# MengRao/pollnet

Hardware: AMD Instinct MI355X
Metric: device-resident Gbit/s + Mframes/s, 1500 B IPv4/TCP frames, 1/2/4/8 MI355X (higher is better)
Workload: dtype u16/u32 integer (one's-complement sums)

## Files before the change

### pollnet_amd/csrc/rx_service.hip

```cpp
#include <algorithm>
#include <chrono>
#include <cstdlib>

#include "rx_classify.hpp"

namespace {
using pn_internal::hip_err;
using pn_internal::set_err;

struct alignas(64) SvcPost {
  uint32_t gen;
  uint32_t n;
  uint32_t fpw;
  uint32_t max_conn;
  const uint8_t* frames;
  pn_result* out;
  const pn_conn_entry* tbl;
  uint16_t* links;
  uint32_t mask;
  uint32_t n_entries;
  uint32_t check;
  uint32_t seq;
};
static_assert(sizeof(SvcPost) == 64, "one line per post");

constexpr uint32_t kDoneWords = 64;
constexpr uint32_t kCountWords = 64;
constexpr uint32_t kExitWord = 96;
constexpr uint32_t kWordsBytes = 512;
constexpr uint32_t kLatWaves = PN_SERVICE_WAVES;
static_assert(kLatWaves <= kDoneWords, "a latency-tier post completes through per-wave done words");
constexpr uint32_t kLatFrames = kLatWaves * kFramesPerWave;
constexpr uint32_t kNetLimitMs = 8000;
constexpr uint32_t kPostVerify = 1u << 30, kPostLinks = 1u << 29, kPostN = (1u << 21) - 1;
constexpr uint32_t kLinkFrames = PN_LINK_MAX_FRAMES, kLinkConns = PN_LINK_MAX_CONNS;
constexpr uint32_t kMailBytes = 4096;

struct alignas(64) SvcDev {
  uint32_t count[2][16];
};
constexpr uint32_t kExitFlag = 32;

#ifdef PN_SVC_TRACE
__device__ uint64_t* g_svc_trace = nullptr;
#define SVC_T(w, i)                                                       \
  do {                                                                    \
    if (lane == 0 && (w) < 64) g_svc_trace[(w) * 8 + (i)] = wall_clock64(); \
  } while (0)
#else
#define SVC_T(w, i) \
  do {              \
  } while (0)
#endif

struct SArgs {
  const SvcPost* mail;
  u32x4* scratch;
  uint32_t* done_words;
  uint32_t* exit_word;
  SvcDev* dev;
  uint64_t idle_ticks;
  uint64_t net_ticks;
  uint32_t epoch;
  uint32_t last;
  uint32_t stride, ipa_off, avail;
  uint32_t poll_sleep;
};

inline uint32_t svc_fpw(uint32_t n, bool verify) {
  uint32_t fpw = verify ? 8u : kFramesPerWave;
  while (fpw < kFramesPerWave && (n + fpw - 1) / fpw > kLatWaves) fpw <<= 1;
  return fpw;
}

inline uint32_t svc_check(const SvcPost* p, uint32_t k) {
  const uint32_t* w = reinterpret_cast<const uint32_t*>(p);
  uint32_t x = k;
  for (int i = 1; i <= 13; i++) x ^= w[i];
  return x;
}

__host__ __device__ __forceinline__ uint32_t svc_active(uint32_t n, uint32_t fpw, uint32_t waves) {
  const uint32_t groups = (n + fpw - 1) / fpw;
  return groups < waves ? groups : waves;
}

inline uint32_t svc_helpers(uint32_t n, uint32_t max) {
  if (n <= kLatFrames) return 0;
  const uint32_t groups = (n + kFramesPerWave - 1) / kFramesPerWave;
  return std::min(groups - kLatWaves, max);
}

__device__ __forceinline__ KArgsAux svc_args(uint32_t v, uint32_t b, const SArgs& s, uint32_t k) {
  auto w32 = [&](uint32_t i) { return (uint32_t)__builtin_amdgcn_readlane(v, b + i); };
  auto u64 = [&](uint32_t lo) { return ((uint64_t)w32(lo + 1) << 32) | w32(lo); };
  KArgsAux a;
  const uint32_t nw = w32(1);
  a.n = nw & kPostN;
  a.fpw = w32(2) & 0xffu;
  a.max_conn = w32(3);
  a.frames = reinterpret_cast<const uint8_t*>(u64(4));
  a.out = reinterpret_cast<pn_result*>(u64(6));
  a.tbl = reinterpret_cast<const pn_conn_entry*>(u64(8));
  a.mask = w32(12);
  a.n_entries = w32(13);
  a.stride = s.stride;
  a.ipa_off = s.ipa_off;
  a.avail = s.avail;
  a.offs = nullptr;
  a.aux = (nw & kPostLinks) ? s.scratch + (size_t)(k & 1) * kLinkFrames * 2 : nullptr;
  return a;
}

__device__ __forceinline__ uint16_t* svc_links(uint32_t v, uint32_t b) {
  return reinterpret_cast<uint16_t*>(((uint64_t)(uint32_t)__builtin_amdgcn_readlane(v, b + 11) << 32) |
                                     (uint32_t)__builtin_amdgcn_readlane(v, b + 10));
}

constexpr uint32_t kCleanNeed = PN_F_HIT | PN_F_ACK | PN_F_IP_OK;
constexpr uint32_t kCleanNone = PN_F_TW | PN_F_SYN | PN_F_FIN | PN_F_RST | PN_F_NOT_TCP | PN_F_TRUNC | PN_F_BADOFF |
                                PN_F_IHL_NE_5;

struct ChainLds {
  uint32_t last[kLinkConns];
  uint32_t key[kLinkFrames];
  uint32_t seq_end[kLinkFrames];
  u32x4 fields[kLinkFrames];
};

__device__ __forceinline__ ChainLds& chain_lds() {
  __shared__ ChainLds c;
  return c;
}

__device__ __forceinline__ void chain_init(int lane) {
  ChainLds& c = chain_lds();
  for (uint32_t i = lane; i < kLinkConns; i += kWave) c.last[i] = 0u;
  wave_lds_sync();
}

__device__ __forceinline__ void chain_step(ChainLds& c, uint32_t base, uint32_t n, uint32_t max_conn, bool on,
                                           const u32x4& rec, const u32x4& fx, const __amdgpu_buffer_rsrc_t& lr,
                                           uint64_t below, int lane) {
  const uint32_t i = base + lane;
  const bool valid = i < n;
  const uint32_t flags = rec.w & 0xffffu;
  const uint32_t len = rec.z >> 16;
  const bool member = on && valid && (flags & (PN_F_HIT | PN_F_TW)) == PN_F_HIT && rec.x < max_conn;
  const bool usable = (flags & kCleanNeed) == kCleanNeed && (flags & kCleanNone) == 0 &&
                      (flags & (PN_F_TCP_OK | PN_F_TCP_UNCHECKED)) != 0 && len != 0 && len < 0x8000u;
  const uint32_t key = member ? rec.x : 0u;
  if (valid) {
    c.key[i] = member ? key : 0xFFFFFFFFu;
    c.seq_end[i] = rec.y + len;
    c.fields[i] = u32x4{fx.x, fx.y, fx.z, (rec.z & 0xffffu) | (usable ? 0x10000u : 0u)};
  }
  uint32_t prev = 0;
  if (member) prev = c.last[key];
  wave_lds_sync();
  if (member) atomicMax(&c.last[key], i + 1);
  wave_lds_sync();
  uint64_t todo = __ballot(member && c.last[key] != i + 1);
  while (todo) {
    const uint32_t leader = (uint32_t)__builtin_ctzll(todo);
    const uint32_t kk = __builtin_amdgcn_readlane(key, leader);
    const uint64_t m = __ballot(member && key == kk);
    todo &= ~m;
    const uint64_t lower = m & below;
    if (member && key == kk && lower) prev = base + 64u - (uint32_t)__builtin_clzll(lower);
  }
  uint32_t d = 0;
  if (member && usable && prev) {
    const uint32_t j = prev - 1;
    const u32x4 pf = c.fields[j];
    if ((pf.w >> 16) && c.seq_end[j] == rec.y && pf.x == fx.x && pf.y == fx.y && pf.z == fx.z &&
        (pf.w & 0xffffu) == (rec.z & 0xffffu))
      d = i - j;
  }
  if (valid) __builtin_amdgcn_raw_buffer_store_b16((unsigned short)d, lr, i * 2, 0, 0);
  wave_lds_sync();
}

__device__ __forceinline__ void chain_pass(const u32x4* aux, uint32_t n, uint32_t max_conn, uint16_t* links, int lane) {
  constexpr int kChunk = 8;
  ChainLds& c = chain_lds();
  const bool on = max_conn <= kLinkConns;
  const __amdgpu_buffer_rsrc_t lr = frame_rsrc(reinterpret_cast<const uint8_t*>(links), n * 2);
  const __amdgpu_buffer_rsrc_t ar = frame_rsrc(reinterpret_cast<const uint8_t*>(aux), n * 32);
  const uint64_t below = (1ull << lane) - 1;
  for (uint32_t base0 = 0; base0 < n; base0 += kChunk * kWave) {
    u32x4 rec[kChunk], fx[kChunk];
#pragma unroll
    for (int s = 0; s < kChunk; ++s) {
      const uint32_t i = base0 + s * kWave + lane;
      rec[s] = __builtin_amdgcn_raw_buffer_load_b128(ar, i * 32, 0, 0);
      fx[s] = __builtin_amdgcn_raw_buffer_load_b128(ar, i * 32 + 16, 0, 0);
    }
#pragma unroll
    for (int s = 0; s < kChunk; ++s)
      if (base0 + s * kWave < n) chain_step(c, base0 + s * kWave, n, max_conn, on, rec[s], fx[s], lr, below, lane);
  }
  for (uint32_t i = lane; i < n; i += kWave) {
    const uint32_t k = c.key[i];
    if (k != 0xFFFFFFFFu) c.last[k] = 0u;
  }
  wave_lds_sync();
}

template <int MIS, int COOP, bool HELPER = false>
__device__ __forceinline__ void svc_run(const KArgsAux& a, bool verify, bool linked, uint32_t w, uint32_t act, uint32_t k,
                                        uint32_t* done_word, int lane) {
  for (uint32_t g = w; g * a.fpw < a.n; g += act) {
    if (verify) classify_group<MIS, COOP, kProdAbl | kChainAux, kLoadAux, kStoreAux, 0, kLoadAux>(a, g * a.fpw, lane);
    else
      classify_group<MIS, COOP, kProdAbl | kHeaderOnly | kChainAux, kLoadAux, kStoreAux, 0, kLoadAux>(a, g * a.fpw, lane);
  }
  if constexpr (HELPER) return;
  __threadfence_system();
  if (lane == 0 && act <= kDoneWords && !linked)
    __hip_atomic_store(done_word, k, __ATOMIC_RELAXED, __HIP_MEMORY_SCOPE_SYSTEM);
}

template <bool PASS>
__device__ __forceinline__ void svc_finish(const KArgsAux& a, uint16_t* links, uint32_t k, uint32_t* count_word, int lane) {
  if constexpr (PASS) {
    if (a.aux) {
      __builtin_amdgcn_fence(__ATOMIC_ACQUIRE, "agent");
      chain_pass(a.aux, a.n, a.max_conn, links, lane);
    }
  }
  __threadfence_system();
  if (lane == 0) __hip_atomic_store(count_word, k, __ATOMIC_RELAXED, __HIP_MEMORY_SCOPE_SYSTEM);
}

template <bool PASS>
__device__ __forceinline__ void svc_count(uint32_t* count, const KArgsAux& a, uint16_t* links, uint32_t target, uint32_t k,
                                          uint32_t* count_word, int lane) {
  uint32_t prev = 0;
  if (lane == 0) prev = atomicAdd(count, 1u);
  prev = __builtin_amdgcn_readfirstlane(prev);
  if (prev == target - 1) {
    if (lane == 0) __hip_atomic_store(count, 0u, __ATOMIC_RELAXED, __HIP_MEMORY_SCOPE_AGENT);
    svc_finish<PASS>(a, links, k, count_word, lane);
  }
}

template <int MIS, int COOP>
__global__ __launch_bounds__(kWave) void rx_service_kernel(SArgs s) {
  const int lane = threadIdx.x;
  const uint32_t w = blockIdx.x, W = gridDim.x;
  const uint32_t* mw = reinterpret_cast<const uint32_t*>(s.mail);
  uint32_t last = s.last;
  uint64_t t0 = wall_clock64();
  chain_init(lane);
  for (;;) {
    const uint32_t v = lane <= (int)kExitFlag ? __hip_atomic_load(mw + lane, __ATOMIC_RELAXED, __HIP_MEMORY_SCOPE_SYSTEM) : 0u;
    if (w != 0 && (uint32_t)__builtin_amdgcn_readlane(v, kExitFlag) == s.epoch) return;
    const uint32_t k = last + 1;
    const uint32_t b = (k & 1) * 16;
    const uint32_t q = __builtin_amdgcn_readlane(v, b + 15);
    uint32_t x = q;
#pragma unroll
    for (uint32_t i = 1; i <= 13; i++) x ^= (uint32_t)__builtin_amdgcn_readlane(v, b + i);
    const bool whole = (uint32_t)__builtin_amdgcn_readlane(v, b) == q && (uint32_t)__builtin_amdgcn_readlane(v, b + 14) == x;
    if (!whole || (int32_t)(q - k) < 0) {
      if (w == 0) {
        if (wall_clock64() - t0 > s.idle_ticks) {
          if (lane == 0) {
            __hip_atomic_store(const_cast<uint32_t*>(mw) + kExitFlag, s.epoch, __ATOMIC_RELAXED, __HIP_MEMORY_SCOPE_SYSTEM);
            __hip_atomic_store(s.exit_word, s.epoch, __ATOMIC_RELEASE, __HIP_MEMORY_SCOPE_SYSTEM);
          }
          return;
        }
        __builtin_amdgcn_s_sleep(1);
      } else {
        if (wall_clock64() - t0 > s.net_ticks) return;
        for (uint32_t i = 0; i < s.poll_sleep; ++i) __builtin_amdgcn_s_sleep(1);
      }
      continue;
    }
    if (q != k) {
      last = k;
      t0 = wall_clock64();
      continue;
    }
    const uint32_t nw = __builtin_amdgcn_readlane(v, b + 1);
    if (nw == PN_SERVICE_STOP) return;
    last = k;
    const uint32_t fw = __builtin_amdgcn_readlane(v, b + 2);
    const uint32_t act = svc_active(nw & kPostN, fw & 0xffu, W + (fw >> 8));
    if (w < act) {
      SVC_T(w, 0);
      __builtin_amdgcn_fence(__ATOMIC_ACQUIRE, "");
      SVC_T(w, 1);
      const KArgsAux a = svc_args(v, b, s, k);
      SVC_T(w, 5);
      const bool linked = a.aux != nullptr;
      svc_run<MIS, COOP>(a, (nw & kPostVerify) != 0, linked, w, act, k, s.done_words + w, lane);
      SVC_T(w, 6);
      if (act > kDoneWords || linked) {
        uint32_t* cw = s.done_words + kCountWords + (k & 1);
        if (act == 1) svc_finish<true>(a, svc_links(v, b), k, cw, lane);
        else svc_count<true>(&s.dev->count[k & 1][0], a, svc_links(v, b), act < W ? act : W, k, cw, lane);
      }
      SVC_T(w, 7);
    }
    t0 = wall_clock64();
  }
}

template <int MIS, int COOP>
__global__ __launch_bounds__(kWave) void rx_service_helper_kernel(KArgsAux a, uint32_t verify, uint32_t act) {
  svc_run<MIS, COOP, true>(a, verify != 0, false, kLatWaves + blockIdx.x, act, 0, nullptr, threadIdx.x);
}

template <int MIS>
void launch_svc(bool coop, uint32_t waves, const SArgs& a, hipStream_t s) {
  if (coop) hipLaunchKernelGGL((rx_service_kernel<MIS, 1>), dim3(waves), dim3(kWave), 0, s, a);
  else hipLaunchKernelGGL((rx_service_kernel<MIS, 0>), dim3(waves), dim3(kWave), 0, s, a);
}

template <int MIS>
void launch_helpers(bool coop, uint32_t helpers, const KArgsAux& a, uint32_t verify, uint32_t act, hipStream_t s) {
  if (coop) hipLaunchKernelGGL((rx_service_helper_kernel<MIS, 1>), dim3(helpers), dim3(kWave), 0, s, a, verify, act);
  else hipLaunchKernelGGL((rx_service_helper_kernel<MIS, 0>), dim3(helpers), dim3(kWave), 0, s, a, verify, act);
}
}

struct pn_service {
  pn_ctx* ctx = nullptr;
  hipStream_t stream = nullptr;
  hipStream_t helper_stream = nullptr;
  uint32_t stride = 0, frame_off = 0;
  uint32_t helpers_max = 0;
  uint32_t post_helpers[2] = {0, 0};
  hipEvent_t helper_ev[2] = {nullptr, nullptr};
  uint64_t idle_ticks = 0, net_ticks = 0;
  SvcPost* mail = nullptr;
  bool mail_dev = false;
  uint32_t* words = nullptr;
  uint32_t post_words[2] = {0, 0};
  uint32_t tbl_post[2] = {0, 0};
  bool tbl_used[2] = {false, false};
  SvcDev* dev = nullptr;
  u32x4* scratch = nullptr;
  uint32_t seq = 0;
  uint32_t epoch = 0;
  bool running = false;
  bool coop = false;
};

namespace {
SArgs svc_sargs(const pn_service* v, uint32_t base) {
  SArgs a;
  a.mail = v->mail;
  a.scratch = v->scratch;
  a.done_words = v->words;
  a.exit_word = v->words + kExitWord;
  a.dev = v->dev;
  a.idle_ticks = v->idle_ticks;
  a.net_ticks = v->net_ticks;
  a.epoch = v->epoch;
  a.last = base;
  a.stride = v->stride;
  a.ipa_off = (v->frame_off + 14) & ~15u;
  a.avail = v->stride - v->frame_off;
  a.poll_sleep = v->mail_dev ? 1u : 16u;
  return a;
}

inline void host_sfence() { asm volatile("sfence" ::: "memory"); }

void svc_publish(SvcPost* slot, const SvcPost& q, bool wc) {
  static const bool avx = __builtin_cpu_supports("avx");
  if (wc && avx) {
    asm volatile(
        "vmovdqu (%0), %%ymm0\n\t"
        "vmovdqu 32(%0), %%ymm1\n\t"
        "vmovntdq %%ymm0, (%1)\n\t"
        "vmovntdq %%ymm1, 32(%1)\n\t"
        "sfence\n\t"
        "vzeroupper"
        :
        : "r"(&q), "r"(slot)
        : "memory", "xmm0", "xmm1");
    return;
  }
  volatile uint32_t* d = reinterpret_cast<volatile uint32_t*>(slot);
  const uint32_t* w = reinterpret_cast<const uint32_t*>(&q);
  for (int i = 1; i <= 14; ++i) d[i] = w[i];
  host_sfence();
  d[0] = w[0];
  d[15] = w[15];
  host_sfence();
}

int svc_launch_helpers(pn_service* v, uint32_t k, uint32_t helpers, const SvcPost& q) {
  KArgsAux a;
  strided_kargs(a, q.frames, q.out, q.tbl, q.mask, q.n_entries, q.max_conn, q.n & kPostN, v->stride, v->frame_off);
  a.fpw = q.fpw & 0xffu;
  const uint32_t verify = (q.n & kPostVerify) ? 1u : 0u, act = svc_active(a.n, a.fpw, kLatWaves + helpers);
  hipStream_t s = v->helper_stream;
  for_mis(v->frame_off, [&](auto mis) { launch_helpers<mis()>(v->coop, helpers, a, verify, act, s); });
  hipError_t e = hipGetLastError();
  if (e == hipSuccess && !v->helper_ev[k & 1]) e = hipEventCreateWithFlags(&v->helper_ev[k & 1], hipEventDisableTiming);
  if (e == hipSuccess) e = hipEventRecord(v->helper_ev[k & 1], s);
  if (e != hipSuccess) return hip_err(v->ctx, e, "pn_service: helper launch");
  return PN_OK;
}

int svc_launch(pn_service* v, uint32_t base) {
  pn_ctx* ctx = v->ctx;
  const SvcDev init{};
  hipError_t e = hipMemcpyAsync(v->dev, &init, sizeof(SvcDev), hipMemcpyHostToDevice, v->stream);
  if (e == hipSuccess) e = hipStreamSynchronize(v->stream);
  if (e != hipSuccess) return hip_err(ctx, e, "pn_service: device state");
  if (++v->epoch == 0) ++v->epoch;
  const SArgs a = svc_sargs(v, base);
  for_mis(v->frame_off, [&](auto mis) { launch_svc<mis()>(v->coop, kLatWaves, a, v->stream); });
  e = hipGetLastError();
  if (e != hipSuccess) return hip_err(ctx, e, "pn_service: launch");
  v->running = true;
  return PN_OK;
}

bool svc_post_ran(const pn_service* v, uint32_t k) {
  const uint32_t words = v->post_words[k & 1];
  if (words == 0 && (int32_t)(__atomic_load_n(v->words + kCountWords + (k & 1), __ATOMIC_ACQUIRE) - k) < 0) return false;
  for (uint32_t w = 0; w < words; ++w)
    if ((int32_t)(__atomic_load_n(v->words + w, __ATOMIC_ACQUIRE) - k) < 0) return false;
  if (v->post_helpers[k & 1] && hipEventQuery(v->helper_ev[k & 1]) != hipSuccess) return false;
  return true;
}

bool svc_post_done(const pn_service* v, uint32_t k) {
  if ((int32_t)(v->seq - k) >= 2) return true;
  if (!svc_post_ran(v, k)) return false;
  return k != v->seq || svc_post_ran(v, k - 1);
}

uint32_t svc_done(const pn_service* v) {
  if (svc_post_done(v, v->seq)) return v->seq;
  return svc_post_done(v, v->seq - 1) ? v->seq - 1 : v->seq - 2;
}

bool svc_exited(const pn_service* v) { return __atomic_load_n(v->words + kExitWord, __ATOMIC_ACQUIRE) == v->epoch; }

void svc_free(pn_service* v) {
  if (v->ctx) {
    auto& l = v->ctx->services;
    l.erase(std::remove(l.begin(), l.end(), v), l.end());
  }
  if (v->mail) (void)(v->mail_dev ? hipFree(v->mail) : hipHostFree(v->mail));
  if (v->words) (void)hipHostFree(v->words);
  if (v->dev) (void)hipFree(v->dev);
  if (v->scratch) (void)hipFree(v->scratch);
  if (v->stream) (void)hipStreamDestroy(v->stream);
  if (v->helper_stream) (void)hipStreamDestroy(v->helper_stream);
  for (hipEvent_t ev : v->helper_ev)
    if (ev) (void)hipEventDestroy(ev);
  delete v;
}
}

int pn_internal::svc_release_table(pn_ctx* ctx, int buf) {
  for (pn_service* v : ctx->services) {
    if (!v->tbl_used[buf]) continue;
    const uint32_t id = v->tbl_post[buf];
    if ((int32_t)(v->seq - id) < 2 && !svc_post_done(v, id)) {
      const int rc = pn_service_wait(v, id);
      if (rc) return rc;
    }
    v->tbl_used[buf] = false;
  }
  return PN_OK;
}

extern "C" {

int pn_service_open(pn_ctx* ctx, uint32_t slot_stride, uint32_t frame_off, uint32_t idle_ms, pn_service** out) {
  return pn_service_open_ex(ctx, slot_stride, frame_off, idle_ms, 0, out);
}

int pn_service_open_ex(pn_ctx* ctx, uint32_t slot_stride, uint32_t frame_off, uint32_t idle_ms, uint32_t large_waves,
                       pn_service** out) {
  if (!ctx || !out) return set_err(ctx, PN_EINVAL, "pn_service_open: ctx / out is NULL");
  *out = nullptr;
  if ((slot_stride & 15) || slot_stride > 65536 || (frame_off & 1) || slot_stride < frame_off + 96)
    return set_err(ctx, PN_EINVAL, "pn_service_open: slot_stride/frame_off violate the layout contract");
  if (idle_ms == 0 || idle_ms > 10000) return set_err(ctx, PN_EINVAL, "pn_service_open: idle_ms must be in [1, 10000]");
  if (large_waves && (large_waves < PN_SERVICE_WAVES || large_waves > PN_SERVICE_MAX_WAVES))
    return set_err(ctx, PN_EINVAL, "pn_service_open: large_waves must be 0 or in [PN_SERVICE_WAVES, PN_SERVICE_MAX_WAVES]");
  hipError_t e = hipSetDevice(ctx->device);
  if (e != hipSuccess) return hip_err(ctx, e, "hipSetDevice");
  int khz = 0;
  e = hipDeviceGetAttribute(&khz, hipDeviceAttributeWallClockRate, ctx->device);
  if (e != hipSuccess || khz <= 0) return hip_err(ctx, e, "pn_service_open: wall clock rate");
  int cus = 0;
  e = hipDeviceGetAttribute(&cus, hipDeviceAttributeMultiprocessorCount, ctx->device);
  if (e != hipSuccess || cus <= 0) return hip_err(ctx, e, "pn_service_open: CU count");
  pn_service* v = new pn_service();
  v->ctx = ctx;
  v->stride = slot_stride;
  v->frame_off = frame_off;
  const uint32_t total = large_waves ? large_waves
                                     : std::max<uint32_t>(kLatWaves, std::min<uint32_t>(PN_SERVICE_MAX_WAVES,
                                                                                      (uint32_t)cus * PN_SERVICE_WAVES_PER_CU));
  v->helpers_max = total - kLatWaves;
  v->idle_ticks = (uint64_t)khz * idle_ms;
  v->net_ticks = v->idle_ticks + (v->idle_ticks >> 1) + (uint64_t)khz * kNetLimitMs;
  v->coop = (slot_stride % 16) == 0 && ((frame_off + 14) & ~15u) >= 16;
  int large_bar = 0;
  if (hipDeviceGetAttribute(&large_bar, hipDeviceAttributeIsLargeBar, ctx->device) != hipSuccess) large_bar = 0;
  v->mail_dev = large_bar != 0 && std::getenv("PN_SERVICE_HOST_MAILBOX") == nullptr;
  if (v->mail_dev && hipExtMallocWithFlags((void**)&v->mail, kMailBytes, hipDeviceMallocUncached) != hipSuccess) {
    (void)hipGetLastError();
    v->mail = nullptr;
    v->mail_dev = false;
  }
  if ((e = hipStreamCreateWithFlags(&v->stream, hipStreamNonBlocking)) != hipSuccess ||
      (e = hipStreamCreateWithFlags(&v->helper_stream, hipStreamNonBlocking)) != hipSuccess ||
      (!v->mail && (e = hipHostMalloc((void**)&v->mail, kMailBytes, hipHostMallocDefault)) != hipSuccess) ||
      (e = hipHostMalloc((void**)&v->words, kWordsBytes, hipHostMallocDefault)) != hipSuccess ||
      (e = hipMalloc((void**)&v->dev, sizeof(SvcDev))) != hipSuccess ||
      (e = hipMalloc((void**)&v->scratch, sizeof(u32x4) * 2 * 2 * kLinkFrames)) != hipSuccess) {
    const int rc = hip_err(ctx, e, "pn_service_open: allocation");
    svc_free(v);
    return rc;
  }
  uint32_t first = 0;
  if (const char* env = std::getenv("PN_SERVICE_FIRST_POST")) first = (uint32_t)std::strtoull(env, nullptr, 0);
  std::memset(v->words, 0, kWordsBytes);
  for (uint32_t w = 0; w < kDoneWords + 2; ++w) v->words[w] = first;
  {
    SvcPost q{};
    q.gen = q.seq = first;
    q.check = ~svc_check(&q, first);
    for (int i = 0; i < 2; ++i) svc_publish(v->mail + i, q, v->mail_dev);
    volatile uint32_t* flag = reinterpret_cast<volatile uint32_t*>(v->mail) + kExitFlag;
    *flag = 0u;
    host_sfence();
  }
  v->seq = first;
  const int rc = svc_launch(v, first);
  if (rc) {
    svc_free(v);
    return rc;
  }
  ctx->services.push_back(v);
  *out = v;
  return PN_OK;
}

int pn_service_post(pn_service* v, const void* frames, uint32_t n, void* results, uint32_t* post_id) {
  return pn_service_post_linked(v, frames, n, results, nullptr, post_id);
}

int pn_service_post_linked(pn_service* v, const void* frames, uint32_t n, void* results, uint16_t* links,
                           uint32_t* post_id) {
  if (!v) return set_err(nullptr, PN_EINVAL, "pn_service_post: service is NULL");
  pn_ctx* ctx = v->ctx;
  if (!ctx->tbl_dev) return set_err(ctx, PN_ENOTABLE, "pn_service_post: no conn table (call pn_set_conn_table)");
  if (n == 0 || n > PN_SERVICE_MAX_FRAMES || !frames || !results)
    return set_err(ctx, PN_EINVAL, "pn_service_post: n must be in [1, PN_SERVICE_MAX_FRAMES], buffers set");
  if (((uintptr_t)frames & 15) || ((uintptr_t)results & 15))
    return set_err(ctx, PN_EINVAL, "pn_service_post: frames/results must be 16-byte aligned");
  if (links && (n > PN_LINK_MAX_FRAMES || ((uintptr_t)links & 1)))
    return set_err(ctx, PN_EINVAL, "pn_service_post_linked: n must be <= PN_LINK_MAX_FRAMES, links 2-byte aligned");
  const uint32_t done = svc_done(v);
  if ((int32_t)(v->seq - done) >= 2) return set_err(ctx, PN_EINVAL, "pn_service_post: two posts already outstanding");
  if (v->running && svc_exited(v)) v->running = false;
  if (!v->running) {
    const int rc = svc_launch(v, done);
    if (rc) return rc;
  }
  const uint32_t k = v->seq + 1;
  const bool verify = ctx->verify_tcp;
  SvcPost q{};
  q.n = n | (verify ? kPostVerify : 0u) | (links ? kPostLinks : 0u);
  q.max_conn = ctx->max_conn;
  q.frames = (const uint8_t*)frames;
  q.out = (pn_result*)results;
  q.tbl = ctx->tbl_dev;
  q.links = links;
  q.mask = (uint32_t)ctx->mask;
  q.n_entries = ctx->n_entries;
  const uint32_t fpw = svc_fpw(n, verify), helpers = svc_helpers(n, v->helpers_max);
  q.fpw = fpw | helpers << 8;
  const uint32_t act = svc_active(n, fpw, kLatWaves + helpers);
  if (helpers) {
    const int rc = svc_launch_helpers(v, k, helpers, q);
    if (rc) return rc;
  }
  v->post_helpers[k & 1] = helpers;
  v->post_words[k & 1] = (act <= kDoneWords && !links) ? act : 0u;
  v->tbl_post[ctx->cur] = k;
  v->tbl_used[ctx->cur] = true;
  q.check = svc_check(&q, k);
  q.gen = q.seq = k;
  svc_publish(v->mail + (k & 1), q, v->mail_dev);
  v->seq = k;
  if (post_id) *post_id = k;
  return PN_OK;
}

int pn_service_wait(pn_service* v, uint32_t post_id) {
  if (!v) return set_err(nullptr, PN_EINVAL, "pn_service_wait: service is NULL");
  if (post_id == 0 || (int32_t)(post_id - v->seq) > 0 || (int32_t)(v->seq - post_id) >= 2)
    post_id = v->seq;
  const uint32_t k = post_id;
  const auto t_start = std::chrono::steady_clock::now();
  for (uint64_t i = 1;; ++i) {
    if (svc_post_done(v, k)) return PN_OK;
    if ((i & 4095) == 0) {
      if (std::chrono::steady_clock::now() - t_start > std::chrono::seconds(10))
        return set_err(v->ctx, PN_EHIP, "pn_service_wait: no completion within 10 s");
      if (svc_exited(v)) {
        const uint32_t done = svc_done(v);
        if ((int32_t)(done - k) >= 0) return PN_OK;
        v->running = false;
        const int rc = svc_launch(v, done);
        if (rc) return rc;
        continue;
      }
      const hipError_t q = hipStreamQuery(v->stream);
      if (q != hipErrorNotReady && q != hipSuccess) return hip_err(v->ctx, q, "pn_service_wait: the service kernel failed");
      if (q == hipSuccess && !svc_post_done(v, k) && !svc_exited(v))
        return set_err(v->ctx, PN_EHIP, "pn_service_wait: the service kernel ended without completing the post");
    }
  }
}

int pn_service_close(pn_service* v) {
  if (!v) return PN_OK;
  pn_ctx* ctx = v->ctx;
  int rc = svc_post_done(v, v->seq) ? PN_OK : pn_service_wait(v, 0);
  if (v->running && !svc_exited(v)) {
    const uint32_t k = v->seq + 1;
    SvcPost q{};
    q.n = PN_SERVICE_STOP;
    v->post_words[k & 1] = 0;
    v->post_helpers[k & 1] = 0;
    q.check = svc_check(&q, k);
    q.gen = q.seq = k;
    svc_publish(v->mail + (k & 1), q, v->mail_dev);
    v->seq = k;
  }
  hipError_t e = hipStreamSynchronize(v->stream);
  if (e == hipSuccess) e = hipStreamSynchronize(v->helper_stream);
  if (e != hipSuccess && rc == PN_OK) rc = hip_err(ctx, e, "pn_service_close");
  svc_free(v);
  return rc;
}

}

#ifdef PN_SVC_TRACE
extern "C" int pn_svc_trace_set(uint64_t* host_buf) {
  return hipMemcpyToSymbol(HIP_SYMBOL(g_svc_trace), &host_buf, sizeof host_buf) == hipSuccess ? PN_OK : PN_EHIP;
}
#endif
```

Before: 51120.

## Launch one helper block per frame group instead of a capped persistent helper grid

The helper kernel used to be a capped set of waves that each looped over frame groups in strided order. It now launches one block per remaining group, in slices, with XCD-aware group mapping and a higher occupancy launch bound. It also drops the chain-aux flag from helper classification and adds propagation of helper errors. The aim is to remove the loop overhead and load imbalance of the persistent helper waves, at the cost of more blocks and possibly several launches for very large posts.

Result: no change. 51120 (-0.0%).

```diff
diff --git a/pollnet_amd/csrc/rx_service.hip b/pollnet_amd/csrc/rx_service.hip
--- a/pollnet_amd/csrc/rx_service.hip
+++ b/pollnet_amd/csrc/rx_service.hip
@@ -85,10 +85,9 @@
   return groups < waves ? groups : waves;
 }
 
-inline uint32_t svc_helpers(uint32_t n, uint32_t max) {
-  if (n <= kLatFrames) return 0;
-  const uint32_t groups = (n + kFramesPerWave - 1) / kFramesPerWave;
-  return std::min(groups - kLatWaves, max);
+inline uint32_t svc_helpers(uint32_t n, bool tier_only) {
+  if (n <= kLatFrames || tier_only) return 0;
+  return (n + kFramesPerWave - 1) / kFramesPerWave - kLatWaves;
 }
 
 __device__ __forceinline__ KArgsAux svc_args(uint32_t v, uint32_t b, const SArgs& s, uint32_t k) {
@@ -207,7 +206,7 @@
   wave_lds_sync();
 }
 
-template <int MIS, int COOP, bool HELPER = false>
+template <int MIS, int COOP>
 __device__ __forceinline__ void svc_run(const KArgsAux& a, bool verify, bool linked, uint32_t w, uint32_t act, uint32_t k,
                                         uint32_t* done_word, int lane) {
   for (uint32_t g = w; g * a.fpw < a.n; g += act) {
@@ -215,7 +214,6 @@
     else
       classify_group<MIS, COOP, kProdAbl | kHeaderOnly | kChainAux, kLoadAux, kStoreAux, 0, kLoadAux>(a, g * a.fpw, lane);
   }
-  if constexpr (HELPER) return;
   __threadfence_system();
   if (lane == 0 && act <= kDoneWords && !linked)
     __hip_atomic_store(done_word, k, __ATOMIC_RELAXED, __HIP_MEMORY_SCOPE_SYSTEM);
@@ -310,8 +308,10 @@
 }
 
 template <int MIS, int COOP>
-__global__ __launch_bounds__(kWave) void rx_service_helper_kernel(KArgsAux a, uint32_t verify, uint32_t act) {
-  svc_run<MIS, COOP, true>(a, verify != 0, false, kLatWaves + blockIdx.x, act, 0, nullptr, threadIdx.x);
+__global__ __launch_bounds__(kWave, 4) void rx_service_helper_kernel(KArgs a, uint32_t verify, uint32_t first) {
+  const uint32_t base = (first + xcd_group(blockIdx.x, gridDim.x)) * a.fpw;
+  if (verify) classify_group<MIS, COOP, kProdAbl, kLoadAux, kStoreAux, 0, kLoadAux>(a, base, threadIdx.x);
+  else classify_group<MIS, COOP, kProdAbl | kHeaderOnly, kLoadAux, kStoreAux, 0, kLoadAux>(a, base, threadIdx.x);
 }
 
 template <int MIS>
@@ -321,9 +321,9 @@
 }
 
 template <int MIS>
-void launch_helpers(bool coop, uint32_t helpers, const KArgsAux& a, uint32_t verify, uint32_t act, hipStream_t s) {
-  if (coop) hipLaunchKernelGGL((rx_service_helper_kernel<MIS, 1>), dim3(helpers), dim3(kWave), 0, s, a, verify, act);
-  else hipLaunchKernelGGL((rx_service_helper_kernel<MIS, 0>), dim3(helpers), dim3(kWave), 0, s, a, verify, act);
+void launch_helpers(bool coop, uint32_t groups, const KArgs& a, uint32_t verify, uint32_t first, hipStream_t s) {
+  if (coop) hipLaunchKernelGGL((rx_service_helper_kernel<MIS, 1>), dim3(groups), dim3(kWave), 0, s, a, verify, first);
+  else hipLaunchKernelGGL((rx_service_helper_kernel<MIS, 0>), dim3(groups), dim3(kWave), 0, s, a, verify, first);
 }
 }
 
@@ -332,9 +332,10 @@
   hipStream_t stream = nullptr;
   hipStream_t helper_stream = nullptr;
   uint32_t stride = 0, frame_off = 0;
-  uint32_t helpers_max = 0;
+  uint32_t helper_slice = 0;
   uint32_t post_helpers[2] = {0, 0};
   hipEvent_t helper_ev[2] = {nullptr, nullptr};
+  mutable hipError_t helper_err = hipSuccess;
   uint64_t idle_ticks = 0, net_ticks = 0;
   SvcPost* mail = nullptr;
   bool mail_dev = false;
@@ -396,12 +397,15 @@
 }
 
 int svc_launch_helpers(pn_service* v, uint32_t k, uint32_t helpers, const SvcPost& q) {
-  KArgsAux a;
+  KArgs a;
   strided_kargs(a, q.frames, q.out, q.tbl, q.mask, q.n_entries, q.max_conn, q.n & kPostN, v->stride, v->frame_off);
   a.fpw = q.fpw & 0xffu;
-  const uint32_t verify = (q.n & kPostVerify) ? 1u : 0u, act = svc_active(a.n, a.fpw, kLatWaves + helpers);
+  const uint32_t verify = (q.n & kPostVerify) ? 1u : 0u;
   hipStream_t s = v->helper_stream;
-  for_mis(v->frame_off, [&](auto mis) { launch_helpers<mis()>(v->coop, helpers, a, verify, act, s); });
+  for (uint32_t g0 = 0; g0 < helpers; g0 += v->helper_slice) {
+    const uint32_t groups = std::min(v->helper_slice, helpers - g0);
+    for_mis(v->frame_off, [&](auto mis) { launch_helpers<mis()>(v->coop, groups, a, verify, kLatWaves + g0, s); });
+  }
   hipError_t e = hipGetLastError();
   if (e == hipSuccess && !v->helper_ev[k & 1]) e = hipEventCreateWithFlags(&v->helper_ev[k & 1], hipEventDisableTiming);
   if (e == hipSuccess) e = hipEventRecord(v->helper_ev[k & 1], s);
@@ -429,7 +433,13 @@
   if (words == 0 && (int32_t)(__atomic_load_n(v->words + kCountWords + (k & 1), __ATOMIC_ACQUIRE) - k) < 0) return false;
   for (uint32_t w = 0; w < words; ++w)
     if ((int32_t)(__atomic_load_n(v->words + w, __ATOMIC_ACQUIRE) - k) < 0) return false;
-  if (v->post_helpers[k & 1] && hipEventQuery(v->helper_ev[k & 1]) != hipSuccess) return false;
+  if (v->post_helpers[k & 1]) {
+    const hipError_t e = hipEventQuery(v->helper_ev[k & 1]);
+    if (e != hipSuccess) {
+      if (e != hipErrorNotReady) v->helper_err = e;
+      return false;
+    }
+  }
   return true;
 }
 
@@ -496,17 +506,11 @@
   int khz = 0;
   e = hipDeviceGetAttribute(&khz, hipDeviceAttributeWallClockRate, ctx->device);
   if (e != hipSuccess || khz <= 0) return hip_err(ctx, e, "pn_service_open: wall clock rate");
-  int cus = 0;
-  e = hipDeviceGetAttribute(&cus, hipDeviceAttributeMultiprocessorCount, ctx->device);
-  if (e != hipSuccess || cus <= 0) return hip_err(ctx, e, "pn_service_open: CU count");
   pn_service* v = new pn_service();
   v->ctx = ctx;
   v->stride = slot_stride;
   v->frame_off = frame_off;
-  const uint32_t total = large_waves ? large_waves
-                                     : std::max<uint32_t>(kLatWaves, std::min<uint32_t>(PN_SERVICE_MAX_WAVES,
-                                                                                      (uint32_t)cus * PN_SERVICE_WAVES_PER_CU));
-  v->helpers_max = total - kLatWaves;
+  v->helper_slice = large_waves ? large_waves - kLatWaves : PN_SERVICE_MAX_FRAMES / kFramesPerWave;
   v->idle_ticks = (uint64_t)khz * idle_ms;
   v->net_ticks = v->idle_ticks + (v->idle_ticks >> 1) + (uint64_t)khz * kNetLimitMs;
   v->coop = (slot_stride % 16) == 0 && ((frame_off + 14) & ~15u) >= 16;
@@ -585,7 +589,7 @@
   q.links = links;
   q.mask = (uint32_t)ctx->mask;
   q.n_entries = ctx->n_entries;
-  const uint32_t fpw = svc_fpw(n, verify), helpers = svc_helpers(n, v->helpers_max);
+  const uint32_t fpw = svc_fpw(n, verify), helpers = svc_helpers(n, v->helper_slice == 0);
   q.fpw = fpw | helpers << 8;
   const uint32_t act = svc_active(n, fpw, kLatWaves + helpers);
   if (helpers) {
@@ -612,6 +616,7 @@
   const auto t_start = std::chrono::steady_clock::now();
   for (uint64_t i = 1;; ++i) {
     if (svc_post_done(v, k)) return PN_OK;
+    if (v->helper_err != hipSuccess) return hip_err(v->ctx, v->helper_err, "pn_service_wait: a large post's helper grid failed");
     if ((i & 4095) == 0) {
       if (std::chrono::steady_clock::now() - t_start > std::chrono::seconds(10))
         return set_err(v->ctx, PN_EHIP, "pn_service_wait: no completion within 10 s");
```
